# MIT-SPARK/Khronos

Measured on AMD Instinct MI355X. Metric: active-window frames/sec (+ Mvoxel-updates/sec) at 1280x720 RGB-D+labels, 2 cm voxels, higher is better.
Workload: dtype f32

## Files before the change

### include/khronos_amd.h

```cpp
#ifndef KHRONOS_AMD_H_
#define KHRONOS_AMD_H_

#include <stddef.h>
#include <stdint.h>

#ifdef __cplusplus
extern "C" {
#endif

#define KHR_OK 0
#define KHR_EINVAL (-1)
#define KHR_ENOMEM (-2)
#define KHR_EDEVICE (-3)
#define KHR_ENOTFOUND (-4)
#define KHR_ESTATE (-5)

#define KHR_VOX_ACTIVE 1u
#define KHR_VOX_EVER_FREE 2u
#define KHR_VOX_TO_REMOVE 4u
#define KHR_VOX_SEM_VALID 8u
#define KHR_BLK_UPDATED 1u
#define KHR_BLK_MESH_UPDATED 2u
#define KHR_BLK_TRACKING_UPDATED 4u
#define KHR_BLK_HAS_ACTIVE_DATA 8u
// ... 160 lines not shown
int khr_detect_objects_launch(khr_ctx* ctx, int slot);
int khr_get_semantic_clusters(khr_ctx* ctx, int slot, khr_cluster* out, int cap);
int64_t khr_cluster_voxels(khr_ctx* ctx, int slot, int which, float voxel_size, int32_t* ids_out, int64_t* voxels_out,
                           int64_t cap);
int khr_cluster_voxels_launch(khr_ctx* ctx, int slot, int which, float voxel_size);
int64_t khr_cluster_voxels_fetch(khr_ctx* ctx, int which, int32_t* ids_out, int64_t* voxels_out, int64_t cap);
typedef struct khr_pixel_ref {
  int32_t slot;
  int32_t which;
  int32_t id;
} khr_pixel_ref;
int khr_pixel_iou(khr_ctx* ctx, int slot, const khr_pixel_ref* refs, int n_refs, int max_id, uint32_t* n_points, uint32_t* inter);
int khr_forward_instances(khr_ctx* ctx, int slot, float max_range, const int32_t* background_ids, int n_background, int max_id,
                          khr_cluster* out);
int khr_generate_mesh(khr_ctx* ctx, int only_mesh_updated, int clear_flag);
#define KHR_MESH_HALO_RECORD_BYTES(vps) (4 * (4 + 3 * 6 * (vps) * (vps)))
int khr_mesh_halo_requests(khr_ctx* ctx, void* keys_out, int64_t cap, int only_mesh_updated, int on_device);
int khr_mesh_halo_export(khr_ctx* ctx, const void* requests, int64_t n_requests, void* records, int64_t cap_records,
                         int on_device);
int khr_mesh_halo_import(khr_ctx* ctx, const void* records, int64_t n_records, int on_device);
#define KHR_MESH_HALO_REQ_HEADER_WORDS(world) (8 * (world))
int khr_mesh_halo_requests_sorted(khr_ctx* ctx, void* requests_device, int64_t cap, int only_mesh_updated);
int khr_mesh_halo_plan(int world, int rank, int vps, const uint64_t* headers, uint64_t* sendcounts, uint64_t* sdispls,
                       uint64_t* recvcounts, uint64_t* rdispls);
int khr_mesh_halo_answer(khr_ctx* ctx, const void* all_requests_device, int64_t cap, const uint64_t* headers, void* records_device,
                         int64_t cap_words);
int khr_mesh_halo_adopt(khr_ctx* ctx, const void* own_requests_device, const uint64_t* own_header, const void* records_device,
                        const uint64_t* rdispls);
int khr_reset_inactive(khr_ctx* ctx, int32_t* removed, int64_t cap, int64_t* n_removed);
int khr_last_removed(khr_ctx* ctx, int32_t* removed, int64_t cap, int64_t* n_removed);
// ... 196 lines not shown
```

### khronos_amd/capi.py

```python
import ctypes as C
import os

import numpy as np

_HERE = os.path.dirname(os.path.abspath(__file__))
LIB_PATH = os.path.join(_HERE, "lib", "libkhronos_amd.so")

KHR_OK, KHR_EINVAL, KHR_ENOMEM, KHR_EDEVICE, KHR_ENOTFOUND, KHR_ESTATE = 0, -1, -2, -3, -4, -5
VOX_ACTIVE, VOX_EVER_FREE, VOX_TO_REMOVE, VOX_SEM_VALID = 1, 2, 4, 8
BLK_UPDATED, BLK_MESH_UPDATED, BLK_TRACKING_UPDATED, BLK_HAS_ACTIVE_DATA = 1, 2, 4, 8


class KhrConfig(C.Structure):
    _fields_ = [
        ("voxel_size", C.c_float), ("voxels_per_side", C.c_int32), ("truncation_distance", C.c_float),
        ("with_semantics", C.c_int32), ("with_tracking", C.c_int32), ("num_labels", C.c_int32),
        ("use_weight_dropoff", C.c_int32), ("weight_dropoff_epsilon", C.c_float),
        ("use_constant_weight", C.c_int32), ("max_weight", C.c_float), ("interpolation_method", C.c_int32),
        ("adaptive_max_range_difference", C.c_float), ("range_mode", C.c_int32), ("semantic_mode", C.c_int32),
        ("label_confidence", C.c_float),
        ("temporal_buffer", C.c_float), ("tsdf_occupancy_threshold", C.c_float),
        ("neighbor_connectivity", C.c_int32), ("temporal_window", C.c_float),
        ("md_neighbor_connectivity", C.c_int32), ("md_min_cluster_size", C.c_int32),
        ("md_max_cluster_size", C.c_int32), ("md_min_separation_distance", C.c_float),
# ... 81 lines not shown

class KhrStats(C.Structure):
    _fields_ = [(n, C.c_uint64) for n in (
        "n_allocated_blocks", "n_visible_blocks", "n_new_blocks", "n_visited_voxels", "n_updated_voxels",
        "n_band_voxels", "n_tracking_updated_blocks", "n_seeds", "n_mesh_blocks", "n_mesh_vertices",
        "pool_exhausted", "cum_updated_voxels", "cum_band_voxels", "cum_visited_voxels", "cum_integrate_calls", "n_tsdf_blocks", "band_overflow",
        "n_tracking_processed_blocks", "n_fuse_items", "n_seed_waits", "n_seed_waits_late", "seed_wait_max_us")] + [
        ("seed_wait_hist", C.c_uint64 * 8)] + [(n, C.c_uint64) for n in (
        "seed_wait_late_us", "seed_wait_late_frame", "seed_wait_late_state", "n_md_device_merges", "n_md_host_walks",
        "n_md_prelaunched", "n_md_prelaunch_repeats")]


EXPORTS = [
    "khr_create", "khr_destroy", "khr_last_error", "khr_host_trace", "khr_set_stream", "khr_sync", "khr_default_config",
    "khr_upload_frame", "khr_set_frame_image", "khr_download_frame", "khr_frame_copy_create", "khr_frame_copy_download", "khr_frame_copy_release", "khr_integrate", "khr_update_tracking",
    "khr_detect_motion", "khr_generate_mesh", "khr_reset_inactive", "khr_mark_all_inactive", "khr_clear_updated",
    "khr_allocate_blocks", "khr_object_prune", "khr_get_stats", "khr_num_blocks", "khr_block_indices",
    "khr_download_block", "khr_mesh_num_vertices", "khr_download_mesh", "khr_fetch_mesh", "khr_fetch_mesh_into", "khr_timing_enable", "khr_timing_reset",
    "khr_timing_get", "khr_debug_read", "khr_tick_ingest", "khr_tick_integrate", "khr_tick_live_bound", "khr_tick_seed_counts", "khr_converted_bytes", "khr_export_converted",
    "khr_converted_views", "khr_tick_adopt", "khr_copy_frame_image", "khr_rv_detect_changes", "khr_last_removed", "khr_process_frame", "khr_ingest_ahead", "khr_ingest_ahead_host", "khr_ingest_cancel", "khr_integrate_shared", "khr_integrate_shared_batch", "khr_pixel_iou", "khr_forward_instances", "khr_update_tracking_phase",
    "khr_export_halo", "khr_import_halo", "khr_get_dynamic_clusters", "khr_motion_keys", "khr_motion_bits_bytes", "khr_motion_bits", "khr_detect_motion_from_bits",
    "khr_dynamic_pack_bytes", "khr_dynamic_unpack_bytes",
    "khr_detect_motion_from_keys", "khr_download_updated", "khr_mesh_halo_requests", "khr_mesh_halo_export",
    "khr_mesh_halo_requests_sorted", "khr_mesh_halo_plan", "khr_mesh_halo_answer", "khr_mesh_halo_adopt",
    "khr_mesh_halo_import", "khr_configure_object_detector", "khr_detect_objects", "khr_get_semantic_clusters",
    "khr_cluster_voxels", "khr_download_frame_image", "khr_detect_objects_launch", "khr_pool_exhausted", "khr_map_digest",
    "khr_rv_create", "khr_rv_destroy", "khr_rv_clear", "khr_rv_add_rays", "khr_rv_num_rays", "khr_rv_num_pairs", "khr_rv_check",
    "khr_snapshot_updated", "khr_take_snapshot", "khr_snapshot_num_blocks", "khr_snapshot_download", "khr_snapshot_download_extra", "khr_snapshot_download_begin", "khr_snapshot_download_end", "khr_snapshot_poll", "khr_fetch_mesh_launch", "khr_reserve_mesh_staging", "khr_reserve_snapshots", "khr_mirror_dynamic", "khr_snapshot_release",
    "khr_rv_check_stamps", "khr_get_config", "khr_cluster_voxels_launch", "khr_cluster_voxels_fetch", "khr_reset_map", "khr_depend_on", "khr_retain_slot", "khr_release_slot",
    "khr_map_slice", "khr_slice_voxel_z", "khr_render_view", "khr_query_points",
    "khr_align_linearize", "khr_align_frame",
# ... 59 lines not shown
    lib.khr_rv_check.argtypes = [vp, C.c_int64, vp, vp, vp, vp, vp, C.POINTER(C.c_uint64), C.POINTER(C.c_uint64)]
    lib.khr_rv_check_stamps.argtypes = [vp, vp, vp]
    lib.khr_rv_detect_changes.argtypes = [vp, C.c_float, C.c_int64, i32, C.c_float, C.c_float, vp, i32, vp, vp, vp]
    lib.khr_get_config.argtypes = [vp, vp]
    lib.khr_reset_map.argtypes = [vp, C.c_float, C.c_float]
    lib.khr_depend_on.argtypes = [vp, vp]
    lib.khr_retain_slot.argtypes = [vp, i32]
    lib.khr_release_slot.argtypes = [vp, i32]
    lib.khr_cluster_voxels_launch.argtypes = [vp, i32, i32, C.c_float]
    lib.khr_cluster_voxels_fetch.argtypes = [vp, i32, vp, vp, C.c_int64]
    lib.khr_cluster_voxels_fetch.restype = C.c_int64
    lib.khr_get_semantic_clusters.argtypes = [vp, i32, C.POINTER(KhrCluster), i32]
    lib.khr_cluster_voxels.argtypes = [vp, i32, i32, C.c_float, vp, vp, C.c_int64]
    lib.khr_cluster_voxels.restype = C.c_int64
    lib.khr_generate_mesh.argtypes = [vp, i32, i32]
    lib.khr_reset_inactive.argtypes = [vp, vp, i64, C.POINTER(i64)]
    lib.khr_mark_all_inactive.argtypes = [vp]
    lib.khr_clear_updated.argtypes = [vp]
    lib.khr_allocate_blocks.argtypes = [vp, vp, i64]
    lib.khr_object_prune.argtypes = [vp, C.c_float, C.c_float, C.POINTER(i64)]
    lib.khr_get_stats.argtypes = [vp, C.POINTER(KhrStats)]
    lib.khr_num_blocks.argtypes = [vp]
    lib.khr_num_blocks.restype = i64
    lib.khr_block_indices.argtypes = [vp, vp, i64, i32]
    lib.khr_block_indices.restype = i64
    lib.khr_download_block.argtypes = [vp, C.c_int32, C.c_int32, C.c_int32] + [vp] * 9
    lib.khr_map_slice.argtypes = [vp, i64, i64] + [vp] * 7
    lib.khr_slice_voxel_z.argtypes = [C.c_float, C.c_float, C.c_int32, vp]
    lib.khr_render_view.argtypes = [vp, C.POINTER(KhrRenderRequest), i32] + [vp] * 6 + [C.POINTER(KhrRenderStats)]
    lib.khr_query_points.argtypes = [vp, i64, vp, C.c_float, i32] + [vp] * 8 + [C.POINTER(KhrQueryStats)]
# ... 950 lines not shown
```

### khronos_amd/csrc/khr_kernels_aux.h

```cpp
#pragma once
#include <cstring>

#include "khr_device.h"

namespace khr {

#include "mc_table.inc"
__device__ int8_t g_mc_tri[256][16];
__device__ uint8_t g_mc_ntri[256];

constexpr uint64_t kSeedBit = kSeedFlag;

__global__ __launch_bounds__(256) void k_motion_pixels(DevMap m, DevParams p, DevFrame f, float md_max_range,
                                                      float min_z_world, uint64_t* __restrict__ keys, int ignore_epoch,
                                                      uint32_t* __restrict__ begin_band_count) {
  if (begin_band_count && blockIdx.x == 0) beginIntegrate(m, p.nvox, begin_band_count);
  const int i = blockIdx.x * blockDim.x + threadIdx.x;
  const bool in = i < f.W * f.H;
  uint64_t key = ~0ull;
  if (in)
    key = motionPixelKey(m, p, f.range[i], f.depth[i], i % f.W, i / f.W, f.fx, f.fy, f.cx, f.cy, f.Rw, f.tw, md_max_range,
                         min_z_world, ignore_epoch);
  if (in) keys[i] = key;
  const bool seed = (key != ~0ull) && (key & kSeedBit);
// ... 921 lines not shown
      const size_t so = static_cast<size_t>(old_offset[s]) + (i - first);
      const float px = s_pts[3 * so], py = s_pts[3 * so + 1], pz = s_pts[3 * so + 2];
      const uint32_t cc = s_col[so], ll = s_lab[so];
      const uint64_t st = s_stm[so];
      d_pts[3 * static_cast<size_t>(i)] = px;
      d_pts[3 * static_cast<size_t>(i) + 1] = py;
      d_pts[3 * static_cast<size_t>(i) + 2] = pz;
      d_col[i] = cc;
      d_lab[i] = ll;
      d_stm[i] = st;
      if (i == first) m.mesh_desc[s].offset = first;
    }
  }
}

template <int VPS, bool EMIT>
__global__ __launch_bounds__(256) void k_marching_cubes(DevMap m, DevParams p, const uint32_t* __restrict__ work,
                                                       const uint32_t* __restrict__ n_work,
                                                       uint32_t* __restrict__ new_count,
                                                       const uint32_t* __restrict__ new_offset, MeshBuffers out,
                                                       int clear_flag, uint32_t max_vertices, RemoteMeshHalo rh,
                                                       uint32_t n_mc_wgs = 0xffffffffu, const uint8_t* __restrict__ regen = nullptr,
                                                       MeshBuffers move_src = MeshBuffers{}, const uint32_t* __restrict__ old_offset = nullptr) {
  constexpr int NV = VPS * VPS * VPS;
  using MH = MeshHalo<VPS>;
  if (EMIT && blockIdx.x >= n_mc_wgs) {
    meshMoveBlocks(m, regen, new_offset, old_offset, move_src, out, max_vertices, blockIdx.x - n_mc_wgs, gridDim.x - n_mc_wgs);
    return;
  }
  const uint32_t mc_grid = min(gridDim.x, n_mc_wgs);
  if (EMIT && new_offset[m.capacity] > max_vertices) {
    if (blockIdx.x == 0 && threadIdx.x == 0) m.counters[C_MESH_OVERFLOW] = 1u;
    return;
  }
  constexpr int T = VPS + 1;
  __shared__ float s_d[T * T * T];
  __shared__ uint8_t s_ok[T * T * T];
  __shared__ uint32_t s_nslot[8];
  __shared__ const uint32_t* s_nrec[8];
  __shared__ int s_nN[8];
  __shared__ uint32_t s_may_cross;
  __shared__ uint32_t s_scan[256];
  __shared__ uint8_t s_ntri[256];
  __shared__ uint16_t s_toff[EMIT ? VPS * VPS * VPS : 2];
  __shared__ uint8_t s_case[EMIT ? VPS * VPS * VPS : 4];
  __shared__ int8_t s_tri[EMIT ? 256 * 16 : 16];
  const uint32_t n = *n_work;
  if (blockIdx.x < n) {
    s_ntri[threadIdx.x] = g_mc_ntri[threadIdx.x];
    if (EMIT)
      reinterpret_cast<uint4*>(s_tri)[threadIdx.x] = reinterpret_cast<const uint4*>(&g_mc_tri[0][0])[threadIdx.x];
  }
  for (uint32_t b = blockIdx.x; b < n; b += mc_grid) {
    const size_t slot = work[b];
    if (EMIT && new_count[slot] == 0u) {
      if (threadIdx.x == 0) {
        m.mesh_desc[slot] = MeshDesc{new_offset[slot], 0u};
        if (clear_flag) atomicAnd(&m.blk_flags[slot], ~BLK_MESH_UPDATED);
      }
      continue;
    }
    const int4 bi = m.blk_index[slot];
    if (threadIdx.x == 0) s_may_cross = 0u;
    __syncthreads();
    if (threadIdx.x < 8) {
      const int k = threadIdx.x;
// ... 33 lines not shown
      int sel = 0;
      if (x >= VPS) { x -= VPS; sel |= 1; }
      if (y >= VPS) { y -= VPS; sel |= 2; }
      if (z >= VPS) { z -= VPS; sel |= 4; }
      const uint32_t ns = s_nslot[sel];
      float d = 0.f, w = -1.f;
      if (ns != kInvalidSlot) {
        const size_t o = static_cast<size_t>(ns) * NV + (x + VPS * (y + VPS * z));
        d = m.dist[o];
        w = m.weight[o];
      } else if (s_nrec[sel]) {
        const int pi = rh.ht_offs ? meshHaloCompactIndex(sel, x, y, z, VPS) : MH::indexOf(sel, x, y, z);
        d = __uint_as_float(s_nrec[sel][pi]);
        w = __uint_as_float(s_nrec[sel][s_nN[sel] + pi]);
      }
      s_d[c] = d;
      s_ok[c] = (w >= p.mesh_min_weight) ? 1 : 0;
    }
    __syncthreads();
    const float ox = static_cast<float>(bi.x) * p.bs, oy = static_cast<float>(bi.y) * p.bs,
                oz = static_cast<float>(bi.z) * p.bs;
    constexpr int PER = NV / 256;
    uint32_t cnt[PER];
    int cases[PER];
    uint32_t tsum = 0;
#pragma unroll
    for (int j = 0; j < PER; ++j) {
      const int lin = threadIdx.x * PER + j;
      const int ix = lin % VPS, iy = (lin / VPS) % VPS, iz = lin / (VPS * VPS);
      int index = 0;
      bool ok = true;
#pragma unroll
      for (int k = 0; k < 8; ++k) {
        const int cx = ix + ((k == 1 || k == 2 || k == 5 || k == 6) ? 1 : 0);
        const int cy = iy + ((k == 2 || k == 3 || k == 6 || k == 7) ? 1 : 0);
        const int cz = iz + (k >= 4 ? 1 : 0);
        const int c = cx + T * (cy + T * cz);
        ok = ok && (s_ok[c] != 0);
        if (s_d[c] < 0.f) index |= (1 << k);
      }
      if (!ok) index = 0;
      cases[j] = index;
      cnt[j] = 3u * s_ntri[index];
      tsum += cnt[j];
    }
    uint32_t incl = tsum;
    {
      const uint32_t ln = threadIdx.x & 63u;
#pragma unroll
      for (int off = 1; off < 64; off <<= 1) {
        const uint32_t up = __shfl_up(incl, off);
        if (ln >= static_cast<uint32_t>(off)) incl += up;
      }
      if (ln == 63u) s_scan[threadIdx.x >> 6] = incl;
    }
    __syncthreads();
    uint32_t wbase = 0, total = 0;
#pragma unroll
    for (uint32_t w = 0; w < 4; ++w) {
      const uint32_t t = s_scan[w];
      if (w < (threadIdx.x >> 6)) wbase += t;
      total += t;
    }
    const uint32_t base = wbase + incl - tsum;
    if (!EMIT) {
      if (threadIdx.x == 0) new_count[slot] = total;
    } else {
      const uint32_t boff = new_offset[slot];
      if (threadIdx.x == 0) {
        m.mesh_desc[slot] = MeshDesc{boff, total};
        if (clear_flag) atomicAnd(&m.blk_flags[slot], ~BLK_MESH_UPDATED);
      }
      {
        uint32_t o = base / 3u;
#pragma unroll
        for (int j = 0; j < PER; ++j) {
          const int lin = threadIdx.x * PER + j;
          s_toff[lin] = static_cast<uint16_t>(o);
          s_case[lin] = static_cast<uint8_t>(cases[j]);
          o += cnt[j] / 3u;
        }
      }
      __syncthreads();
      const uint32_t n_tri = total / 3u;
      float* __restrict__ const o_pts = out.points;
      uint32_t* __restrict__ const o_col = out.colors;
      uint32_t* __restrict__ const o_lab = out.labels;
      uint64_t* __restrict__ const o_stm = out.stamps;
      const uint32_t* __restrict__ const g_col = m.color;
      const uint32_t* __restrict__ const g_lab = m.sem_label;
      const ulonglong2* __restrict__ const g_obs = m.obs;
      const uint64_t* __restrict__ const g_lobs = m.last_obs;
      for (uint32_t tri = threadIdx.x; tri < n_tri; tri += 256) {
        int lo = 0, hi = NV - 1;
        while (lo < hi) {
          const int mid = (lo + hi + 1) >> 1;
          if (s_toff[mid] <= tri) lo = mid; else hi = mid - 1;
        }
        const int lin = lo;
        const int index = s_case[lin];
        const int col = 3 * static_cast<int>(tri - s_toff[lin]);
        const int ix = lin % VPS, iy = (lin / VPS) % VPS, iz = lin / (VPS * VPS);
        float vp[3][3];
        uint32_t vcol[3], vlab[3];
        uint64_t vstm[3];
        ulonglong2 vobs[3];
        size_t vso[3];
        bool vlocal[3];
#pragma unroll
        for (int kk = 2; kk >= 0; --kk) {
          const int e = s_tri[index * 16 + col + kk];
          const int ea = (e < 8) ? e : (e - 8);
          const int eb = (e < 4) ? ((e + 1) & 3) : (e < 8 ? 4 + ((e - 4 + 1) & 3) : e - 4);
          const int ax = (ea == 1 || ea == 2 || ea == 5 || ea == 6), ay = (ea == 2 || ea == 3 || ea == 6 || ea == 7),
                    az = ea >= 4;
          const int bx = (eb == 1 || eb == 2 || eb == 5 || eb == 6), by = (eb == 2 || eb == 3 || eb == 6 || eb == 7),
                    bz = eb >= 4;
          const float s0 = s_d[(ix + ax) + T * ((iy + ay) + T * (iz + az))];
          const float s1 = s_d[(ix + bx) + T * ((iy + by) + T * (iz + bz))];
          const float diff = s0 - s1;
          float t = 0.5f;
          if (fabsf(diff) >= p.mesh_eps) t = s0 / diff;
          const float p0x = ox + (static_cast<float>(ix + ax) + 0.5f) * p.vs;
          const float p0y = oy + (static_cast<float>(iy + ay) + 0.5f) * p.vs;
          const float p0z = oz + (static_cast<float>(iz + az) + 0.5f) * p.vs;
          const float p1x = ox + (static_cast<float>(ix + bx) + 0.5f) * p.vs;
// ... 37 lines not shown
          if (vlocal[kk] && p.with_tracking) {
            const uint32_t bit = static_cast<uint32_t>(vso[kk]) & 63u;
            vstm[kk] = ((vobs[kk].x >> bit) & 1ull) ? vobs[kk].y : g_lobs[vso[kk]];
          }
        }
#pragma unroll
        for (int kk = 2; kk >= 0; --kk) {
          const size_t vo = static_cast<size_t>(boff) + 3u * tri + static_cast<uint32_t>(2 - kk);
          o_pts[3 * vo] = vp[kk][0];
          o_pts[3 * vo + 1] = vp[kk][1];
          o_pts[3 * vo + 2] = vp[kk][2];
          o_col[vo] = vcol[kk];
          o_lab[vo] = vlab[kk];
          o_stm[vo] = vstm[kk];
        }
      }
    }
  }
}

__global__ __launch_bounds__(256) void k_mesh_halo_requests(DevMap m, DevParams p, const uint32_t* __restrict__ work,
                                                           const uint32_t* __restrict__ n_work, uint64_t* __restrict__ req,
                                                           uint32_t cap, uint32_t* __restrict__ n_req) {
  const uint32_t n = *n_work;
  for (uint32_t i = blockIdx.x * blockDim.x + threadIdx.x; i < ((n * 7 + 63) / 64) * 64; i += gridDim.x * blockDim.x) {
    bool want = false;
    uint64_t key = 0;
    if (i < n * 7) {
      const int4 bi = m.blk_index[work[i / 7]];
      const int k = static_cast<int>(i % 7) + 1;
// ... 197 lines not shown
      listed = (fl & require_flags) == require_flags;
      const MeshDesc d = m.mesh_desc[s];
      count = d.count;
      offset = d.offset;
    }
  }
  if (s < m.capacity) old_offset[s] = offset;
  const uint32_t idx = waveAggInc(n_work, listed);
  if (listed) work[idx] = s;
  if (s <= m.capacity) {
    if (s < m.capacity) regen[s] = listed ? 1 : 0;
    new_count[s] = count;
  }
}

__global__ __launch_bounds__(256) void k_mesh_carry_counts(DevMap m, uint32_t* __restrict__ new_count) {
  const uint32_t s = blockIdx.x * blockDim.x + threadIdx.x;
  if (s >= m.counters[C_MAX_SLOT]) return;
  new_count[s] = (m.blk_flags[s] & BLK_LIVE) ? m.mesh_desc[s].count : 0u;
}

__global__ __launch_bounds__(256) void k_mark_regen(const uint32_t* __restrict__ work, const uint32_t* n_work,
                                                   uint8_t* __restrict__ regen) {
  const uint32_t i = blockIdx.x * blockDim.x + threadIdx.x;
  if (i < *n_work) regen[work[i]] = 1;
}

template <int VPS>
__global__ __launch_bounds__(256) void k_reset_inactive(DevMap m, int4* __restrict__ removed, uint32_t clear_mask) {
  const uint32_t n_slots = m.counters[C_MAX_SLOT];
// ... 329 lines not shown
```

### khronos_amd/csrc/khronos_amd.hip

```cpp
#include <hip/hip_runtime.h>
#include <hip/hip_ext.h>
#include <hipcub/hipcub.hpp>

#include <algorithm>
#include <array>
#include <atomic>
#include <chrono>
#include <memory>
#include <mutex>
#include <cmath>
#include <cstdarg>
#include <cstdio>
#include <climits>
#include <cstring>
#include <cstdlib>
#include <functional>
#include <map>
#include <string>
#include <thread>
#include <tuple>
#include <unordered_map>
#include <vector>

#include "../../include/khronos_amd.h"
// ... 199 lines not shown
  int ef_parity = 0, ef_cur = 0;
  hipEvent_t ev_seed = nullptr;
  uint32_t last_removed = 0;
  khr_ctx* dep_src = nullptr;
  hipEvent_t ev_dep = nullptr, ev_dep_aux = nullptr;
  uint64_t last_track_stamp = 0;
  bool removed_pending = false;
  int4* d_removed = nullptr;
  int4* h_removed_early = nullptr;
  uint32_t* d_removed_early_n = nullptr;
  uint32_t removed_early_ticket = 0;
  bool removed_early = false;
  int* d_idx_staging = nullptr;
  uint64_t* d_keys = nullptr;
  uint32_t* d_pix = nullptr;
  void* d_cub_temp = nullptr;
  uint64_t* d_md_keys = nullptr;
  uint32_t *d_md_counts = nullptr, *d_md_ids = nullptr, *d_md_n = nullptr, *d_md_adj = nullptr;
  uint64_t *d_md_seed_keys = nullptr, *d_md_bnd_keys = nullptr;
  uint32_t *d_md_seed_counts = nullptr, *d_md_bnd_counts = nullptr;
  int32_t *d_md_seed_final = nullptr, *d_md_bnd_final = nullptr;
  int32_t* d_md_bnd_deg = nullptr;
  unsigned long long* d_md_bnd_mask = nullptr;
  uint64_t n_seed_waits = 0, n_seed_waits_late = 0, seed_wait_max_us = 0, seed_wait_hist[8] = {0, 0, 0, 0, 0, 0, 0, 0};
  uint64_t seed_wait_late_us = 0, seed_wait_late_frame = 0, seed_wait_late_state = 0;
  bool last_ingest_on_aux = false;
  uint64_t n_md_device_merges = 0, n_md_host_walks = 0;
  std::vector<int32_t> h_md_bnd_deg;
  ClusterAcc* d_md_acc = nullptr;
  uint32_t *d_md_parent = nullptr, *d_md_rootidx = nullptr;
  CompAcc* d_md_comp_acc = nullptr;
// ... 11 lines not shown
  uint32_t md_last_seeds = 0;
  uint8_t* d_md_head_host = nullptr;
  uint32_t* d_md_edges = nullptr;
  uint32_t* d_md_scratch4 = nullptr;
  std::vector<uint64_t> h_md_seed_keys, h_md_bnd_keys;
  std::vector<uint32_t> h_md_seed_counts, h_md_bnd_counts, h_md_adj;
  uint32_t* h_md_walk = nullptr;
  size_t h_md_walk_words = 0;
  hipEvent_t ev_md_walk_up = nullptr;
  std::vector<int32_t> h_md_seed_final, h_md_bnd_final;
  std::vector<ClusterAcc> h_md_acc;
  ClusterAcc* h_md_acc_pinned = nullptr;
  ClusterAcc* d_md_acc_host = nullptr;
  uint32_t md_acc_ticket = 0;
  int md_acc_slot = -1;
  size_t cub_temp_bytes = 0;
  bool obj_configured = false;
  khr_object_detector_config obj_cfg{};
  std::vector<int32_t> obj_labels;
  int32_t* d_obj_labels = nullptr;
  uint64_t* d_gv_keys = nullptr;
  uint32_t gv_mask = 0;
  uint32_t *d_gv_parent = nullptr, *d_gv_rootidx = nullptr, *d_gv_node = nullptr, *d_gv_n = nullptr;
  ObjAcc* d_obj_acc = nullptr;
  int32_t* d_obj_final = nullptr;
  uint64_t* d_cv_list = nullptr;
  uint32_t obj_root_cap = 0;
  uint32_t* d_gv_owners = nullptr;
  uint32_t* d_gv_done = nullptr;
  bool gv_clean = false;
  bool gv_counters_clean[3] = {false, false, false};
// ... 3 lines not shown
  uint32_t* d_cv_n[2] = {nullptr, nullptr};
  uint64_t* d_cv_keys[2] = {nullptr, nullptr};
  uint8_t* h_cv[2] = {nullptr, nullptr};
  uint8_t* d_cv_host[2] = {nullptr, nullptr};
  uint8_t* d_obj_head_host = nullptr;
  hipEvent_t ev_cv[2] = {nullptr, nullptr};
  int cv_pending_slot[2] = {-1, -1};
  uint32_t obj_ticket = 0, cv_ticket[2] = {0, 0};
  int3 cv_origin[2]{};
  MeshBuffers mesh[2]{};
  int mesh_cur = 0;
  uint32_t *d_mesh_count = nullptr, *d_mesh_offset = nullptr;
  uint8_t* d_regen = nullptr;
  uint32_t* d_mesh_old_off = nullptr;
  uint32_t* d_mesh_nwork = nullptr;
  uint64_t mesh_total = 0;
  bool mesh_stale = false;
  std::vector<uint32_t> h_counters;
  khr_stats stats{};
  bool host_index_valid = false;
  std::map<std::array<int32_t, 3>, uint32_t> host_index;
  std::vector<uint32_t> host_flags;
  uint64_t* d_slice_keys = nullptr;
  uint32_t* d_slice_count = nullptr;
  uint8_t* d_slice_stage = nullptr;
  uint8_t* h_slice_stage = nullptr;
  uint32_t slice_cap = 0, slice_hint = 0;
  unsigned long long* d_render_stats = nullptr;
  uint8_t* d_render_stage = nullptr;
  uint8_t* h_render_stage = nullptr;
// ... 614 lines not shown
    A(devAlloc(c, &c->d_md_adj, static_cast<size_t>(c->md_list_cap) * 26, false));
    {
      const size_t want = std::min<size_t>(c->md_list_cap, 16384) * (3 + 26 + 3) + 16;
      if (hipHostMalloc(reinterpret_cast<void**>(&c->h_md_walk), want * 4, hipHostMallocDefault) != hipSuccess) A(KHR_ENOMEM);
      else c->h_md_walk_words = want;
    }
    A(devAlloc(c, &c->d_md_acc, 256, false));
    if (hipHostMalloc(reinterpret_cast<void**>(&c->h_md_acc_pinned), sizeof(ClusterAcc) * 256, hipHostMallocDefault) != hipSuccess ||
        hipHostGetDevicePointer(reinterpret_cast<void**>(&c->d_md_acc_host), c->h_md_acc_pinned, 0) != hipSuccess)
      A(KHR_ENOMEM);
    {
      std::vector<ClusterAcc> init(256);
      for (auto& a : init) clusterAccReset(a);
      if (rc == KHR_OK && hipMemcpy(c->d_md_acc, init.data(), sizeof(ClusterAcc) * 256, hipMemcpyHostToDevice) != hipSuccess) A(KHR_EDEVICE);
    }
  }
  if (rc == KHR_OK) {
    size_t t3 = 0;
    hipcub::DeviceScan::ExclusiveSum(nullptr, t3, c->d_mesh_count, c->d_mesh_offset, static_cast<int>(cap + 1), c->stream);
    c->cub_temp_bytes = t3 + 256;
    uint8_t* tmp = nullptr;
    A(devAlloc(c, &tmp, c->cub_temp_bytes, false));
    c->d_cub_temp = tmp;
  }
  for (int b = 0; b < 2 && rc == KHR_OK; ++b) {
    A(devAlloc(c, &c->mesh[b].points, cfg->max_mesh_vertices * 3, false));
    A(devAlloc(c, &c->mesh[b].colors, cfg->max_mesh_vertices, false));
    A(devAlloc(c, &c->mesh[b].labels, cfg->max_mesh_vertices, false));
    A(devAlloc(c, &c->mesh[b].stamps, cfg->max_mesh_vertices, false));
  }
  c->slots.resize(cfg->num_frame_slots);
  c->slot_leases.reset(new std::atomic<int>[cfg->num_frame_slots]);
  for (uint32_t i = 0; i < cfg->num_frame_slots; ++i) c->slot_leases[i].store(0);
  for (auto& s : c->slots) {
    if (rc != KHR_OK) break;
    A(devAlloc(c, &s.depth, npx, false));
    A(devAlloc(c, &s.range, npx + 4, false));
    A(devAlloc(c, &s.rgba, npx + 4, false));
// ... 2438 lines not shown
    k.num_pixels_painted = a.n_pixels;
    k.semantic_id = static_cast<int32_t>(id);
    if (a.n_pixels) {
      ++present;
      for (int d = 0; d < 3; ++d) {
        k.bbox_min[d] = orderedToFloat(a.bmin[d]);
        k.bbox_max[d] = orderedToFloat(a.bmax[d]);
        k.centroid[d] = a.sum[d] / static_cast<float>(a.n_pixels);
      }
    }
    out[id] = k;
  }
  return present;
}

int khr_generate_mesh(khr_ctx* c, int only_mesh_updated, int clear_flag) {
  if (!c) return fail(KHR_EINVAL, "null ctx");
  HIP_TRY(hipSetDevice(c->device));
  DevMap& m = c->m;
  const size_t cap = m.capacity;
  ScopedTimer tm(c, 5);
  HIP_TRY(hipMemsetAsync(c->d_mesh_nwork, 0, sizeof(uint32_t), c->stream));
  hipLaunchKernelGGL(k_mesh_prepare, dim3(gridFor(cap + 1)), dim3(256), 0, c->stream, m, only_mesh_updated ? BLK_MESH_UPDATED : 0u,
                     c->d_work, c->d_mesh_nwork, c->d_regen, c->d_mesh_count, c->d_mesh_old_off);
  MeshBuffers src = c->mesh[c->mesh_cur], dst = c->mesh[c->mesh_cur ^ 1];
  RemoteMeshHalo rmh{};
  if (c->mh_n) {
    rmh.recs = c->mh_view;
    rmh.ht_keys = c->d_mh_keys;
    rmh.ht_vals = c->d_mh_vals;
    rmh.ht_mask = c->mh_mask;
    if (c->mh_compact) {
      rmh.ht_keys = c->d_mh2_keys;
      rmh.ht_offs = c->d_mh2_offs;
    }
  }
  const uint32_t maxv = static_cast<uint32_t>(std::min<uint64_t>(c->cfg.max_mesh_vertices, 0xfffffff0ull));
  int rc = dispatchVps(c, [&](auto vps) {
    constexpr int V = decltype(vps)::value;
    KHR_LAUNCH_TIMED(8, (k_marching_cubes<V, false>), dim3(kStreamGrid), dim3(256), m, c->p, c->d_work,
                     c->d_mesh_nwork, c->d_mesh_count, c->d_mesh_offset, dst, clear_flag, maxv, rmh, 0xffffffffu,
                     static_cast<const uint8_t*>(nullptr), MeshBuffers{}, static_cast<const uint32_t*>(nullptr));
    size_t tb = c->cub_temp_bytes;
    HIP_TRY(hipcub::DeviceScan::ExclusiveSum(c->d_cub_temp, tb, c->d_mesh_count, c->d_mesh_offset,
                                             static_cast<int>(cap + 1), c->stream));
    constexpr uint32_t kMoveWgs = 1024;
    KHR_LAUNCH_TIMED(9, (k_marching_cubes<V, true>), dim3(kStreamGrid + kMoveWgs), dim3(256), m, c->p, c->d_work,
                     c->d_mesh_nwork, c->d_mesh_count, c->d_mesh_offset, dst, clear_flag, maxv, rmh, static_cast<uint32_t>(kStreamGrid),
                     static_cast<const uint8_t*>(c->d_regen), src, static_cast<const uint32_t*>(c->d_mesh_old_off));
    return KHR_OK;
  });
  if (rc) return rc;
  c->mesh_cur ^= 1;
  c->mesh_stale = true;
  HIP_TRY(hipGetLastError());
  return KHR_OK;
}

static int removedPublishLaunch(khr_ctx* c) {
  if (!c->h_removed_early) {
    if (hipHostMalloc(reinterpret_cast<void**>(&c->h_removed_early), sizeof(int4) * c->m.capacity, hipHostMallocDefault) != hipSuccess)
      return fail(KHR_ENOMEM, "page-locked list of archived blocks (%zu bytes)", sizeof(int4) * static_cast<size_t>(c->m.capacity));
    int rc = devAlloc(c, &c->d_removed_early_n, 2);
    if (rc) return rc;
  }
  void* list_dev = nullptr;
  HIP_TRY(hipHostGetDevicePointer(&list_dev, c->h_removed_early, 0));
// ... 1791 lines not shown
    if (err & kCkptErrPool) return fail(KHR_ENOMEM, "checkpoint: the block pool (max_blocks %u) ran out during the load", c->m.capacity);
    return fail(KHR_EDEVICE, "checkpoint: %u blocks restored, %llu expected", live, static_cast<unsigned long long>(kept));
  }
  c->host_index_valid = false, ++c->map_gen;
  c->stats = khr_stats{};
  if (n_kept) *n_kept = static_cast<int64_t>(kept);
  return KHR_OK;
}

static int refreshMeshTotals(khr_ctx* c) {
  if (!c->mesh_stale) return KHR_OK;
  if (!c->h_totals && hipHostMalloc(reinterpret_cast<void**>(&c->h_totals), sizeof(uint32_t) * (C_COUNT + 2), hipHostMallocDefault) != hipSuccess)
    return fail(KHR_ENOMEM, "pinned block for the mesh totals");
  uint32_t* hs = c->h_totals;
  HIP_TRY(hipMemcpyAsync(hs, c->d_mesh_offset + c->m.capacity, sizeof(uint32_t), hipMemcpyDeviceToHost, c->stream));
  HIP_TRY(hipMemcpyAsync(hs + 1, c->d_mesh_nwork, sizeof(uint32_t), hipMemcpyDeviceToHost, c->stream));
  HIP_TRY(hipMemcpyAsync(hs + 2, c->m.counters, sizeof(uint32_t) * C_COUNT, hipMemcpyDeviceToHost, c->stream));
  HIP_TRY(hipStreamSynchronize(c->stream));
  const uint32_t total = hs[0], nwork = hs[1];
  c->h_counters.assign(hs + 2, hs + 2 + C_COUNT);
  c->counters_gen = c->map_gen;
  const uint32_t ovf = c->h_counters[C_MESH_OVERFLOW];
  if (ovf) return fail(KHR_ENOMEM, "mesh needs %u vertices, max_mesh_vertices=%llu", total,
                       static_cast<unsigned long long>(c->cfg.max_mesh_vertices));
  c->mesh_total = total;
  c->stats.n_mesh_blocks = nwork;
  c->stats.n_mesh_vertices = total;
  c->mesh_stale = false;
  return KHR_OK;
}

// ... 607 lines not shown
```

Measured before the change: 4039.

## Restructure marching-cubes emission with compact LDS entry lists and custom scan

```diff
diff --git a/include/khronos_amd.h b/include/khronos_amd.h
--- a/include/khronos_amd.h
+++ b/include/khronos_amd.h
@@ -198,6 +198,7 @@
 int khr_forward_instances(khr_ctx* ctx, int slot, float max_range, const int32_t* background_ids, int n_background, int max_id,
                           khr_cluster* out);
 int khr_generate_mesh(khr_ctx* ctx, int only_mesh_updated, int clear_flag);
+int khr_mesh_list_capacity(int voxels_per_side);
 #define KHR_MESH_HALO_RECORD_BYTES(vps) (4 * (4 + 3 * 6 * (vps) * (vps)))
 int khr_mesh_halo_requests(khr_ctx* ctx, void* keys_out, int64_t cap, int only_mesh_updated, int on_device);
 int khr_mesh_halo_export(khr_ctx* ctx, const void* requests, int64_t n_requests, void* records, int64_t cap_records,
diff --git a/khronos_amd/capi.py b/khronos_amd/capi.py
--- a/khronos_amd/capi.py
+++ b/khronos_amd/capi.py
@@ -119,7 +119,7 @@
 EXPORTS = [
     "khr_create", "khr_destroy", "khr_last_error", "khr_host_trace", "khr_set_stream", "khr_sync", "khr_default_config",
     "khr_upload_frame", "khr_set_frame_image", "khr_download_frame", "khr_frame_copy_create", "khr_frame_copy_download", "khr_frame_copy_release", "khr_integrate", "khr_update_tracking",
-    "khr_detect_motion", "khr_generate_mesh", "khr_reset_inactive", "khr_mark_all_inactive", "khr_clear_updated",
+    "khr_detect_motion", "khr_generate_mesh", "khr_mesh_list_capacity", "khr_reset_inactive", "khr_mark_all_inactive", "khr_clear_updated",
     "khr_allocate_blocks", "khr_object_prune", "khr_get_stats", "khr_num_blocks", "khr_block_indices",
     "khr_download_block", "khr_mesh_num_vertices", "khr_download_mesh", "khr_fetch_mesh", "khr_fetch_mesh_into", "khr_timing_enable", "khr_timing_reset",
     "khr_timing_get", "khr_debug_read", "khr_tick_ingest", "khr_tick_integrate", "khr_tick_live_bound", "khr_tick_seed_counts", "khr_converted_bytes", "khr_export_converted",
@@ -209,6 +209,7 @@
     lib.khr_cluster_voxels.argtypes = [vp, i32, i32, C.c_float, vp, vp, C.c_int64]
     lib.khr_cluster_voxels.restype = C.c_int64
     lib.khr_generate_mesh.argtypes = [vp, i32, i32]
+    lib.khr_mesh_list_capacity.argtypes = [i32]
     lib.khr_reset_inactive.argtypes = [vp, vp, i64, C.POINTER(i64)]
     lib.khr_mark_all_inactive.argtypes = [vp]
     lib.khr_clear_updated.argtypes = [vp]
diff --git a/khronos_amd/csrc/khr_kernels_aux.h b/khronos_amd/csrc/khr_kernels_aux.h
--- a/khronos_amd/csrc/khr_kernels_aux.h
+++ b/khronos_amd/csrc/khr_kernels_aux.h
@@ -959,8 +959,11 @@
   }
 }
 
+__host__ __device__ constexpr int kMcListCap(int vps) { return vps >= 16 ? 256 : 128; }
+constexpr uint32_t kMcUnobserved = 0xffffffffu;
+
 template <int VPS, bool EMIT>
-__global__ __launch_bounds__(256) void k_marching_cubes(DevMap m, DevParams p, const uint32_t* __restrict__ work,
+__global__ __launch_bounds__(256, 4) void k_marching_cubes(DevMap m, DevParams p, const uint32_t* __restrict__ work,
                                                        const uint32_t* __restrict__ n_work,
                                                        uint32_t* __restrict__ new_count,
                                                        const uint32_t* __restrict__ new_offset, MeshBuffers out,
@@ -979,22 +982,31 @@
     return;
   }
   constexpr int T = VPS + 1;
+  constexpr int CAP = kMcListCap(VPS);
   __shared__ float s_d[T * T * T];
-  __shared__ uint8_t s_ok[T * T * T];
   __shared__ uint32_t s_nslot[8];
   __shared__ const uint32_t* s_nrec[8];
   __shared__ int s_nN[8];
   __shared__ uint32_t s_may_cross;
-  __shared__ uint32_t s_scan[256];
+  __shared__ uint32_t s_scan[4];
   __shared__ uint8_t s_ntri[256];
-  __shared__ uint16_t s_toff[EMIT ? VPS * VPS * VPS : 2];
-  __shared__ uint8_t s_case[EMIT ? VPS * VPS * VPS : 4];
+  __shared__ uint32_t s_ent[EMIT ? CAP : 1];
+#ifdef KHR_MC_DEAL_ENTRIES
+  __shared__ uint16_t s_etoff[EMIT ? CAP : 2];
+#else
+  __shared__ uint16_t s_t2e[EMIT ? 5 * CAP : 2];
+#endif
+  __shared__ uint32_t s_rbase[EMIT ? NV / CAP + 1 : 1];
+#ifdef KHR_MC_TRI_LDS
   __shared__ int8_t s_tri[EMIT ? 256 * 16 : 16];
+#endif
   const uint32_t n = *n_work;
   if (blockIdx.x < n) {
     s_ntri[threadIdx.x] = g_mc_ntri[threadIdx.x];
+#ifdef KHR_MC_TRI_LDS
     if (EMIT)
       reinterpret_cast<uint4*>(s_tri)[threadIdx.x] = reinterpret_cast<const uint4*>(&g_mc_tri[0][0])[threadIdx.x];
+#endif
   }
   for (uint32_t b = blockIdx.x; b < n; b += mc_grid) {
     const size_t slot = work[b];
@@ -1058,35 +1070,33 @@
         d = __uint_as_float(s_nrec[sel][pi]);
         w = __uint_as_float(s_nrec[sel][s_nN[sel] + pi]);
       }
-      s_d[c] = d;
-      s_ok[c] = (w >= p.mesh_min_weight) ? 1 : 0;
+      s_d[c] = (w >= p.mesh_min_weight) ? d : __uint_as_float(kMcUnobserved);
     }
     __syncthreads();
     const float ox = static_cast<float>(bi.x) * p.bs, oy = static_cast<float>(bi.y) * p.bs,
                 oz = static_cast<float>(bi.z) * p.bs;
     constexpr int PER = NV / 256;
-    uint32_t cnt[PER];
-    int cases[PER];
+    uint32_t cc[(PER + 3) / 4] = {};
     uint32_t tsum = 0;
 #pragma unroll
     for (int j = 0; j < PER; ++j) {
       const int lin = threadIdx.x * PER + j;
       const int ix = lin % VPS, iy = (lin / VPS) % VPS, iz = lin / (VPS * VPS);
-      int index = 0;
+      uint32_t index = 0;
       bool ok = true;
 #pragma unroll
       for (int k = 0; k < 8; ++k) {
         const int cx = ix + ((k == 1 || k == 2 || k == 5 || k == 6) ? 1 : 0);
         const int cy = iy + ((k == 2 || k == 3 || k == 6 || k == 7) ? 1 : 0);
         const int cz = iz + (k >= 4 ? 1 : 0);
-        const int c = cx + T * (cy + T * cz);
-        ok = ok && (s_ok[c] != 0);
-        if (s_d[c] < 0.f) index |= (1 << k);
+        const float d = s_d[cx + T * (cy + T * cz)];
+        ok = ok && (__float_as_uint(d) != kMcUnobserved);
+        if (d < 0.f) index |= (1u << k);
       }
       if (!ok) index = 0;
-      cases[j] = index;
-      cnt[j] = 3u * s_ntri[index];
-      tsum += cnt[j];
+      const uint32_t nt = s_ntri[index];
+      cc[j >> 2] |= index << (8 * (j & 3));
+      tsum += nt + (nt ? 0x10000u : 0u);
     }
     uint32_t incl = tsum;
     {
@@ -1107,26 +1117,15 @@
       total += t;
     }
     const uint32_t base = wbase + incl - tsum;
+    const uint32_t total_tri = total & 0xffffu, total_ne = total >> 16;
     if (!EMIT) {
-      if (threadIdx.x == 0) new_count[slot] = total;
+      if (threadIdx.x == 0) new_count[slot] = 3u * total_tri;
     } else {
       const uint32_t boff = new_offset[slot];
       if (threadIdx.x == 0) {
-        m.mesh_desc[slot] = MeshDesc{boff, total};
+        m.mesh_desc[slot] = MeshDesc{boff, 3u * total_tri};
         if (clear_flag) atomicAnd(&m.blk_flags[slot], ~BLK_MESH_UPDATED);
       }
-      {
-        uint32_t o = base / 3u;
-#pragma unroll
-        for (int j = 0; j < PER; ++j) {
-          const int lin = threadIdx.x * PER + j;
-          s_toff[lin] = static_cast<uint16_t>(o);
-          s_case[lin] = static_cast<uint8_t>(cases[j]);
-          o += cnt[j] / 3u;
-        }
-      }
-      __syncthreads();
-      const uint32_t n_tri = total / 3u;
       float* __restrict__ const o_pts = out.points;
       uint32_t* __restrict__ const o_col = out.colors;
       uint32_t* __restrict__ const o_lab = out.labels;
@@ -1135,15 +1134,7 @@
       const uint32_t* __restrict__ const g_lab = m.sem_label;
       const ulonglong2* __restrict__ const g_obs = m.obs;
       const uint64_t* __restrict__ const g_lobs = m.last_obs;
-      for (uint32_t tri = threadIdx.x; tri < n_tri; tri += 256) {
-        int lo = 0, hi = NV - 1;
-        while (lo < hi) {
-          const int mid = (lo + hi + 1) >> 1;
-          if (s_toff[mid] <= tri) lo = mid; else hi = mid - 1;
-        }
-        const int lin = lo;
-        const int index = s_case[lin];
-        const int col = 3 * static_cast<int>(tri - s_toff[lin]);
+      auto emitTri = [&](const int lin, const int index, const int col, const uint32_t tri) {
         const int ix = lin % VPS, iy = (lin / VPS) % VPS, iz = lin / (VPS * VPS);
         float vp[3][3];
         uint32_t vcol[3], vlab[3];
@@ -1153,7 +1144,11 @@
         bool vlocal[3];
 #pragma unroll
         for (int kk = 2; kk >= 0; --kk) {
+#ifdef KHR_MC_TRI_LDS
           const int e = s_tri[index * 16 + col + kk];
+#else
+          const int e = g_mc_tri[index][col + kk];
+#endif
           const int ea = (e < 8) ? e : (e - 8);
           const int eb = (e < 4) ? ((e + 1) & 3) : (e < 8 ? 4 + ((e - 4 + 1) & 3) : e - 4);
           const int ax = (ea == 1 || ea == 2 || ea == 5 || ea == 6), ay = (ea == 2 || ea == 3 || ea == 6 || ea == 7),
@@ -1221,6 +1216,52 @@
           o_lab[vo] = vlab[kk];
           o_stm[vo] = vstm[kk];
         }
+      };
+      const uint32_t n_rounds = (total_ne + CAP - 1u) / CAP;
+      for (uint32_t r = 0; r < n_rounds; ++r) {
+        const uint32_t r0 = r * CAP;
+        if (r) __syncthreads();
+        const uint32_t rb = r ? s_rbase[r] : 0u;
+        {
+          uint32_t pos = base >> 16, o = base & 0xffffu;
+#pragma unroll
+          for (int j = 0; j < PER; ++j) {
+            const uint32_t index = (cc[j >> 2] >> (8 * (j & 3))) & 0xffu;
+            const uint32_t nt = s_ntri[index];
+            if (nt) {
+              const uint32_t e = pos - r0;
+              if (e < static_cast<uint32_t>(CAP)) {
+                s_ent[e] = static_cast<uint32_t>(threadIdx.x * PER + j) | (index << 12);
+#ifdef KHR_MC_DEAL_ENTRIES
+                s_etoff[e] = static_cast<uint16_t>(o);
+#else
+#pragma unroll 1
+                for (uint32_t t = 0; t < nt; ++t) s_t2e[o - rb + t] = static_cast<uint16_t>((e << 3) | t);
+#endif
+              }
+              if (r == 0u && pos % CAP == 0u) s_rbase[pos / CAP] = o;
+              ++pos;
+              o += nt;
+            }
+          }
+          if (r == 0u && threadIdx.x == 0) s_rbase[n_rounds] = total_tri;
+        }
+        __syncthreads();
+#ifdef KHR_MC_DEAL_ENTRIES
+        const uint32_t n_in = min(static_cast<uint32_t>(CAP), total_ne - r0);
+        for (uint32_t e = threadIdx.x; e < n_in; e += 256) {
+          const uint32_t ent = s_ent[e], first = s_etoff[e];
+          const uint32_t nt = s_ntri[ent >> 12];
+          for (uint32_t t = 0; t < nt; ++t) emitTri(static_cast<int>(ent & 0xfffu), static_cast<int>(ent >> 12), static_cast<int>(3u * t), first + t);
+        }
+#else
+        const uint32_t re = s_rbase[r + 1];
+        for (uint32_t tri = rb + threadIdx.x; tri < re; tri += 256) {
+          const uint32_t te = s_t2e[tri - rb];
+          const uint32_t ent = s_ent[te >> 3];
+          emitTri(static_cast<int>(ent & 0xfffu), static_cast<int>(ent >> 12), static_cast<int>(3u * (te & 7u)), tri);
+        }
+#endif
       }
     }
   }
@@ -1448,6 +1489,56 @@
   }
 }
 
+__global__ __launch_bounds__(1024) void k_mesh_scan(const uint32_t* __restrict__ count, uint32_t* __restrict__ offset, uint32_t n,
+                                                    uint32_t* __restrict__ next_n_work) {
+  __shared__ uint32_t s_wave[2][16];
+  if (threadIdx.x == 0) *next_n_work = 0u;
+  const uint32_t lane = threadIdx.x & 63u, wave = threadIdx.x >> 6;
+  auto load = [&](uint32_t i) {
+    uint4 v = make_uint4(0u, 0u, 0u, 0u);
+    if (i + 4u <= n) {
+      v = *reinterpret_cast<const uint4*>(count + i);
+    } else {
+      if (i < n) v.x = count[i];
+      if (i + 1u < n) v.y = count[i + 1u];
+      if (i + 2u < n) v.z = count[i + 2u];
+    }
+    return v;
+  };
+  uint32_t carry = 0u, round = 0u;
+  uint4 next = load(threadIdx.x * 4u);
+  for (uint32_t base = 0u; base < n; base += 4096u, round ^= 1u) {
+    const uint32_t i = base + threadIdx.x * 4u;
+    const uint4 v = next;
+    if (base + 4096u < n) next = load(i + 4096u);
+    const uint32_t tsum = v.x + v.y + v.z + v.w;
+    uint32_t incl = tsum;
+#pragma unroll
+    for (int off = 1; off < 64; off <<= 1) {
+      const uint32_t up = __shfl_up(incl, off);
+      if (lane >= static_cast<uint32_t>(off)) incl += up;
+    }
+    if (lane == 63u) s_wave[round][wave] = incl;
+    __syncthreads();
+    uint32_t wbase = 0u, total = 0u;
+#pragma unroll
+    for (uint32_t w = 0; w < 16u; ++w) {
+      const uint32_t t = s_wave[round][w];
+      if (w < wave) wbase += t;
+      total += t;
+    }
+    const uint32_t o = carry + wbase + incl - tsum;
+    if (i + 4u <= n) {
+      *reinterpret_cast<uint4*>(offset + i) = make_uint4(o, o + v.x, o + v.x + v.y, o + v.x + v.y + v.z);
+    } else {
+      if (i < n) offset[i] = o;
+      if (i + 1u < n) offset[i + 1u] = o + v.x;
+      if (i + 2u < n) offset[i + 2u] = o + v.x + v.y;
+    }
+    carry += total;
+  }
+}
+
 __global__ __launch_bounds__(256) void k_mesh_carry_counts(DevMap m, uint32_t* __restrict__ new_count) {
   const uint32_t s = blockIdx.x * blockDim.x + threadIdx.x;
   if (s >= m.counters[C_MAX_SLOT]) return;
diff --git a/khronos_amd/csrc/khronos_amd.hip b/khronos_amd/csrc/khronos_amd.hip
--- a/khronos_amd/csrc/khronos_amd.hip
+++ b/khronos_amd/csrc/khronos_amd.hip
@@ -1,6 +1,5 @@
 #include <hip/hip_runtime.h>
 #include <hip/hip_ext.h>
-#include <hipcub/hipcub.hpp>
 
 #include <algorithm>
 #include <array>
@@ -237,7 +236,6 @@
   int* d_idx_staging = nullptr;
   uint64_t* d_keys = nullptr;
   uint32_t* d_pix = nullptr;
-  void* d_cub_temp = nullptr;
   uint64_t* d_md_keys = nullptr;
   uint32_t *d_md_counts = nullptr, *d_md_ids = nullptr, *d_md_n = nullptr, *d_md_adj = nullptr;
   uint64_t *d_md_seed_keys = nullptr, *d_md_bnd_keys = nullptr;
@@ -279,7 +277,6 @@
   ClusterAcc* d_md_acc_host = nullptr;
   uint32_t md_acc_ticket = 0;
   int md_acc_slot = -1;
-  size_t cub_temp_bytes = 0;
   bool obj_configured = false;
   khr_object_detector_config obj_cfg{};
   std::vector<int32_t> obj_labels;
@@ -313,6 +310,7 @@
   uint8_t* d_regen = nullptr;
   uint32_t* d_mesh_old_off = nullptr;
   uint32_t* d_mesh_nwork = nullptr;
+  uint32_t mesh_nwork_next = 0, mesh_nwork_last = 0;
   uint64_t mesh_total = 0;
   bool mesh_stale = false;
   std::vector<uint32_t> h_counters;
@@ -957,14 +955,6 @@
       for (auto& a : init) clusterAccReset(a);
       if (rc == KHR_OK && hipMemcpy(c->d_md_acc, init.data(), sizeof(ClusterAcc) * 256, hipMemcpyHostToDevice) != hipSuccess) A(KHR_EDEVICE);
     }
-  }
-  if (rc == KHR_OK) {
-    size_t t3 = 0;
-    hipcub::DeviceScan::ExclusiveSum(nullptr, t3, c->d_mesh_count, c->d_mesh_offset, static_cast<int>(cap + 1), c->stream);
-    c->cub_temp_bytes = t3 + 256;
-    uint8_t* tmp = nullptr;
-    A(devAlloc(c, &tmp, c->cub_temp_bytes, false));
-    c->d_cub_temp = tmp;
   }
   for (int b = 0; b < 2 && rc == KHR_OK; ++b) {
     A(devAlloc(c, &c->mesh[b].points, cfg->max_mesh_vertices * 3, false));
@@ -3433,15 +3423,21 @@
   return present;
 }
 
+int khr_mesh_list_capacity(int voxels_per_side) {
+  if (voxels_per_side != 8 && voxels_per_side != 16) return fail(KHR_EINVAL, "voxels_per_side must be 8 or 16");
+  return kMcListCap(voxels_per_side);
+}
+
 int khr_generate_mesh(khr_ctx* c, int only_mesh_updated, int clear_flag) {
   if (!c) return fail(KHR_EINVAL, "null ctx");
   HIP_TRY(hipSetDevice(c->device));
   DevMap& m = c->m;
   const size_t cap = m.capacity;
   ScopedTimer tm(c, 5);
-  HIP_TRY(hipMemsetAsync(c->d_mesh_nwork, 0, sizeof(uint32_t), c->stream));
+  uint32_t* const n_work = c->d_mesh_nwork + c->mesh_nwork_next;
+  uint32_t* const n_work_other = c->d_mesh_nwork + (c->mesh_nwork_next ^ 4u);
   hipLaunchKernelGGL(k_mesh_prepare, dim3(gridFor(cap + 1)), dim3(256), 0, c->stream, m, only_mesh_updated ? BLK_MESH_UPDATED : 0u,
-                     c->d_work, c->d_mesh_nwork, c->d_regen, c->d_mesh_count, c->d_mesh_old_off);
+                     c->d_work, n_work, c->d_regen, c->d_mesh_count, c->d_mesh_old_off);
   MeshBuffers src = c->mesh[c->mesh_cur], dst = c->mesh[c->mesh_cur ^ 1];
   RemoteMeshHalo rmh{};
   if (c->mh_n) {
@@ -3458,18 +3454,22 @@
   int rc = dispatchVps(c, [&](auto vps) {
     constexpr int V = decltype(vps)::value;
     KHR_LAUNCH_TIMED(8, (k_marching_cubes<V, false>), dim3(kStreamGrid), dim3(256), m, c->p, c->d_work,
-                     c->d_mesh_nwork, c->d_mesh_count, c->d_mesh_offset, dst, clear_flag, maxv, rmh, 0xffffffffu,
+                     n_work, c->d_mesh_count, c->d_mesh_offset, dst, clear_flag, maxv, rmh, 0xffffffffu,
                      static_cast<const uint8_t*>(nullptr), MeshBuffers{}, static_cast<const uint32_t*>(nullptr));
-    size_t tb = c->cub_temp_bytes;
-    HIP_TRY(hipcub::DeviceScan::ExclusiveSum(c->d_cub_temp, tb, c->d_mesh_count, c->d_mesh_offset,
-                                             static_cast<int>(cap + 1), c->stream));
+    hipLaunchKernelGGL(k_mesh_scan, dim3(1), dim3(1024), 0, c->stream, c->d_mesh_count, c->d_mesh_offset, static_cast<uint32_t>(cap + 1),
+                       n_work_other);
     constexpr uint32_t kMoveWgs = 1024;
     KHR_LAUNCH_TIMED(9, (k_marching_cubes<V, true>), dim3(kStreamGrid + kMoveWgs), dim3(256), m, c->p, c->d_work,
-                     c->d_mesh_nwork, c->d_mesh_count, c->d_mesh_offset, dst, clear_flag, maxv, rmh, static_cast<uint32_t>(kStreamGrid),
+                     n_work, c->d_mesh_count, c->d_mesh_offset, dst, clear_flag, maxv, rmh, static_cast<uint32_t>(kStreamGrid),
                      static_cast<const uint8_t*>(c->d_regen), src, static_cast<const uint32_t*>(c->d_mesh_old_off));
     return KHR_OK;
   });
-  if (rc) return rc;
+  if (rc) {
+    hipMemsetAsync(n_work, 0, sizeof(uint32_t), c->stream);
+    return rc;
+  }
+  c->mesh_nwork_last = c->mesh_nwork_next;
+  c->mesh_nwork_next ^= 4u;
   c->mesh_cur ^= 1;
   c->mesh_stale = true;
   HIP_TRY(hipGetLastError());
@@ -5291,7 +5291,7 @@
     return fail(KHR_ENOMEM, "pinned block for the mesh totals");
   uint32_t* hs = c->h_totals;
   HIP_TRY(hipMemcpyAsync(hs, c->d_mesh_offset + c->m.capacity, sizeof(uint32_t), hipMemcpyDeviceToHost, c->stream));
-  HIP_TRY(hipMemcpyAsync(hs + 1, c->d_mesh_nwork, sizeof(uint32_t), hipMemcpyDeviceToHost, c->stream));
+  HIP_TRY(hipMemcpyAsync(hs + 1, c->d_mesh_nwork + c->mesh_nwork_last, sizeof(uint32_t), hipMemcpyDeviceToHost, c->stream));
   HIP_TRY(hipMemcpyAsync(hs + 2, c->m.counters, sizeof(uint32_t) * C_COUNT, hipMemcpyDeviceToHost, c->stream));
   HIP_TRY(hipStreamSynchronize(c->stream));
   const uint32_t total = hs[0], nwork = hs[1];
```

Measured after the change: 3997. -1.0%, worse.
